# dkogan/mrcal

Hardware: AMD Instinct MI355X
Metric: LM (dog-leg) iterations/sec, 8-cam x 1000-frame OPENCV8 calibration (higher is better)
Workload: dtype f64; 1 GPU; 8 cameras x 1000 frames x 10x10 corners, LENSMODEL_OPENCV8, all variables optimized, warp + regularization; Nstate=6140, Nmeasurements=1600080, Nnz_J=37200080, parallelism=single GPU

## Files before the change

### mrcal_amd/csrc/kernels.hip

```cpp
#include <hip/hip_runtime.h>
#include <utility>
#include <stdlib.h>
#include "problem.hpp"
#include "device_math.hpp"
#include "lens_models.hpp"
#include "lens_dispatch.hpp"
#include "triangulation.hpp"
#include "kernels.hpp"
#include "dogleg_choose.hpp"
#include "kernels_shared.hpp"

namespace mrcal_amd {

__device__ __forceinline__
void joint_pose_record(double* __restrict__ out,
                       const double* rt_cam,
                       const double* rt_frame)
{
    double R[9], dR[27];
    if(rt_cam == NULL)
    {
        R_from_r_with_grad(R, dR, rt_frame);
        for(int i=0;i<9;i++) out[JOINT_R + i] = R[i];
        for(int i=0;i<3;i++) out[JOINT_T + i] = rt_frame[3+i];
// ... 246 lines not shown
        if(c.skip_eval) return;
        board_prologue_body(P, B, dogleg_trial_state(ca, c), ca.ops[c.ia], nblocks_unpack, nblocks_zero, reg_mode);
    }
    else
    {
        if(opref_skip(R)) return;
        const double* b = opref_get(R).b;
        board_prologue_body(P, B, b, opref_get(R), nblocks_unpack, nblocks_zero, reg_mode);
    }
}


__device__ __forceinline__
int board_csr_to_tile_col(const DeviceProblem& P, bool has_ext, int c, int xy)
{
    const int b1 = P.Ncore_state ? 2 : 0;
    const int b2 = b1 + P.Ndist_state;
    const int b3 = b2 + (has_ext ? 6 : 0);
    const int b4 = b3 + (P.do_optimize_frames ? 6 : 0);
    int col = tile_warp0(P.Ndist) + (c - b4);
    col = (c < b4) ? tile_frame0(P.Ndist) + (c - b3) : col;
    col = (c < b3) ? tile_ext0(P.Ndist)   + (c - b2) : col;
    col = (c < b2) ? 4 + (c - b1)                    : col;
    col = (c < b1) ? 2*c + xy                        : col;
    return col;
}

template<int N>
__device__ __forceinline__ double row_ror_f64(double v)
{
    union { double d; int i[2]; } u; u.d = v;
    u.i[0] = __builtin_amdgcn_update_dpp(0, u.i[0], 0x120 + N, 0xf, 0xf, true);
    u.i[1] = __builtin_amdgcn_update_dpp(0, u.i[1], 0x120 + N, 0xf, 0xf, true);
    return u.d;
}

typedef double d2_t __attribute__((ext_vector_type(2)));
typedef __attribute__((address_space(1))) double gdouble;
typedef __attribute__((address_space(1))) d2_t   gdouble2;

typedef double gram_d2 __attribute__((ext_vector_type(2)));
__device__ __forceinline__ gram_d2 lds_read2_b64_16(unsigned lds_byte_address)
{
    gram_d2 v;
    asm volatile("ds_read2_b64 %0, %1 offset1:16" : "=v"(v) : "v"(lds_byte_address) : "memory");
    return v;
}

template<int K, int KS>
__device__ __forceinline__
void copy_out_full(const double* __restrict__ tile, gdouble* __restrict__ out,
                   int A0, int A1, int B0, int B1, unsigned gofs, int rsub)
{
    constexpr int PAIRS = K/2, R = 64/PAIRS;
    constexpr int NIT   = (64 + 2*R - 1)/(2*R);
    const char* __restrict__ t = reinterpret_cast<const char*>(tile);
#pragma unroll
    for(int it0 = 0; it0 < NIT; it0 += 2)
    {
        d2_t v[4];
#pragma unroll
        for(int q=0;q<4;q++)
        {
            const int it = it0 + (q >> 1), u = q & 1;
            const int rb = it*2*R + u*R;
            if(it >= NIT || rb >= 64) continue;
            const int o  = it*2*R*KS*(int)sizeof(double);
            v[q].x = *reinterpret_cast<const double*>(t + (u ? B0 : A0) + o);
            v[q].y = *reinterpret_cast<const double*>(t + (u ? B1 : A1) + o);
        }
#pragma unroll
        for(int q=0;q<4;q++)
        {
            const int it = it0 + (q >> 1), u = q & 1;
            const int rb = it*2*R + u*R;
            if(it >= NIT || rb >= 64) continue;
            gdouble* __restrict__ o = out + rb*K;
            if(rb + R - 1 < 64)      __builtin_nontemporal_store(v[q], reinterpret_cast<gdouble2*>(&o[gofs]));
            else if(rsub < 64 - rb)  __builtin_nontemporal_store(v[q], reinterpret_cast<gdouble2*>(&o[gofs]));
        }
    }
}

template<int NBLK, int MM> struct GramCand
{
    static constexpr int      c    = gram_cand(NBLK, MM);
    static constexpr GramDesc d    = gram_cand_desc(NBLK, c);
    static constexpr bool     roty = gram_rotated_y(NBLK);
    static constexpr int srcA = (d.kind == GRAM_YY) ? 1 : 0;
    static constexpr int srcB = (d.kind == GRAM_XX) ? 0 : (roty ? 1 : 1 + d.q);
    static constexpr int rotB = (d.kind == GRAM_XX || roty) ? d.q : 0;
};
struct GramRd { double v[4]; };
template<int NBLK, int NACC, int... MM>
__device__ __forceinline__ void gram_mfmas(double (&acc)[NACC], const double (&op)[4][4], std::integer_sequence<int, MM...>)
{
    ((acc[MM] = __builtin_amdgcn_mfma_f64_4x4x4f64(op[GramCand<NBLK,MM>::srcA][0],
                                                   op[GramCand<NBLK,MM>::srcB][GramCand<NBLK,MM>::rotB],
                                                   acc[MM], 0, 0, 0)), ...);
}
template<int NBLK, int NM>
__device__ __forceinline__ void gram_step_ops(double (&acc)[NM], const GramRd& rd)
{
    double op[4][4];
#pragma unroll
    for(int g=0; g<4; g++)
    {
        op[g][0] = rd.v[g];
        op[g][1] = row_ror_f64<12>(op[g][0]);
        op[g][2] = row_ror_f64<8 >(op[g][0]);
        op[g][3] = row_ror_f64<4 >(op[g][0]);
    }
    gram_mfmas<NBLK>(acc, op, std::make_integer_sequence<int, NM>{});
}

__device__ __forceinline__ void permlane32_swap_f64(double& a, double& b)
{
    union { double d; unsigned u[2]; } ua, ub;
    ua.d = a; ub.d = b;
#pragma unroll
    for(int i = 0; i < 2; i++)
    {
        const auto r = __builtin_amdgcn_permlane32_swap(ua.u[i], ub.u[i], false, false);
        ua.u[i] = r[0]; ub.u[i] = r[1];
    }
    a = ua.d; b = ub.d;
}

template<int OFF>
__device__ __forceinline__ double lds_read_b64_at(unsigned lds_byte_address)
{
    double v;
    asm volatile("ds_read_b64 %0, %1 offset:%2" : "=v"(v) : "v"(lds_byte_address), "n"(OFF) : "memory");
    return v;
}

template<int NREAD>
__device__ __forceinline__ void lgkm_wait0(GramRd& a, d2_t& b)
{
    if(NREAD == 2)      asm volatile("s_waitcnt lgkmcnt(0)" : "+v"(a.v[0]), "+v"(a.v[1]), "+v"(b) :: "memory");
    else if(NREAD == 3) asm volatile("s_waitcnt lgkmcnt(0)" : "+v"(a.v[0]), "+v"(a.v[1]), "+v"(a.v[2]), "+v"(b) :: "memory");
    else                asm volatile("s_waitcnt lgkmcnt(0)" : "+v"(a.v[0]), "+v"(a.v[1]), "+v"(a.v[2]), "+v"(a.v[3]), "+v"(b) :: "memory");
}
template<int S, bool FULL, bool STORE, int NBLK, int K, int KS, int NM>
__device__ __forceinline__
void fused_step(double (&acc)[NM], GramRd& cur, const unsigned (&gram_a)[4], unsigned tile_a0,
                gdouble* __restrict__ out, int A0, int A1, int B0, int B1, unsigned gofs, int rsub, int nrows)
{
    if(!FULL && 4*S >= nrows) return;
    constexpr int PAIRS = K/2, R = 64/PAIRS, NGRP = (64 + R - 1)/R;
    constexpr int NREAD = gram_nreads(NBLK);
    constexpr bool have_grp = STORE && S < NGRP;
    constexpr int  u  = S & 1;
    constexpr int  go = (S >> 1)*2*R*KS*(int)sizeof(double);
    constexpr int  rb = S*R;
    GramRd nxt = cur;
    if(S < 15)
    {
        constexpr int so = (S < 15 ? S+1 : 0)*(FULL ? 1 : 4)*KS*(int)sizeof(double);
#pragma unroll
        for(int q=0;q<NREAD;q++) nxt.v[q] = lds_read_b64_at<so>(gram_a[q]);
    }
    d2_t v = {0.0, 0.0};
    if(have_grp)
    {
        v.x = lds_read_b64_at<go>(tile_a0 + (unsigned)(u ? B0 : A0));
        v.y = lds_read_b64_at<go>(tile_a0 + (unsigned)(u ? B1 : A1));
    }
    if(S == 0)
    {
        d2_t none = {0.0, 0.0};
        if(!FULL || !have_grp) lgkm_wait0<NREAD>(cur, none);
        else if(NREAD == 2) asm volatile("s_waitcnt lgkmcnt(4)" : "+v"(cur.v[0]), "+v"(cur.v[1]), "+v"(none) :: "memory");
        else if(NREAD == 3) asm volatile("s_waitcnt lgkmcnt(5)" : "+v"(cur.v[0]), "+v"(cur.v[1]), "+v"(cur.v[2]), "+v"(none) :: "memory");
        else                asm volatile("s_waitcnt lgkmcnt(6)" : "+v"(cur.v[0]), "+v"(cur.v[1]), "+v"(cur.v[2]), "+v"(cur.v[3]), "+v"(none) :: "memory");
    }
    __builtin_amdgcn_sched_barrier(0);
    gram_step_ops<NBLK>(acc, cur);
    __builtin_amdgcn_sched_barrier(0);
    lgkm_wait0<NREAD>(nxt, v);
    if(have_grp)
    {
        gdouble* __restrict__ o = out + rb*K;
        if(FULL)
        {
            if(rb + R - 1 < 64)      __builtin_nontemporal_store(v, reinterpret_cast<gdouble2*>(&o[gofs]));
            else if(rsub < 64 - rb)  __builtin_nontemporal_store(v, reinterpret_cast<gdouble2*>(&o[gofs]));
        }
        else if(rb + rsub < nrows)   __builtin_nontemporal_store(v, reinterpret_cast<gdouble2*>(&o[gofs]));
    }
    __builtin_amdgcn_sched_barrier(0);
    cur = nxt;
}
template<bool FULL, bool STORE, int NBLK, int K, int KS, int NM, int... S>
__device__ __forceinline__
void fused_steps(double (&acc)[NM], GramRd& cur, const unsigned (&gram_a)[4], unsigned tile_a0,
                 gdouble* __restrict__ out, int A0, int A1, int B0, int B1, unsigned gofs, int rsub, int nrows,
                 std::integer_sequence<int, S...>)
{
    (fused_step<S,FULL,STORE,NBLK,K,KS>(acc, cur, gram_a, tile_a0, out, A0, A1, B0, B1, gofs, rsub, nrows), ...);
}
template<bool FULL, bool STORE, int NBLK, int K, int KS, int NM>
__device__ __forceinline__
void gram_copy_fused(double (&acc)[NM], const double* __restrict__ tile, const int (&goffs)[4],
                     gdouble* __restrict__ out, int A0, int A1, int B0, int B1, unsigned gofs, int rsub, int nrows)
{
    constexpr int NREAD = gram_nreads(NBLK);
    static_assert(NREAD >= 2 && NREAD <= 4, "board tiles have 5..8 column blocks");
    const unsigned tile_a0 = (unsigned)(size_t)tile;
    const unsigned row_skew = FULL ? (unsigned)((threadIdx.x >> 4)*15*KS*sizeof(double)) : 0u;
    unsigned gram_a[4];
#pragma unroll
    for(int q=0;q<4;q++) gram_a[q] = tile_a0 + row_skew + (unsigned)(goffs[q < NREAD ? q : 0]*sizeof(double));
    GramRd cur;
#pragma unroll
    for(int q=0;q<4;q++) cur.v[q] = 0.0;
#pragma unroll
    for(int q=0;q<NREAD;q++) cur.v[q] = lds_read_b64_at<0>(gram_a[q]);
    fused_steps<FULL,STORE,NBLK,K,KS>(acc, cur, gram_a, tile_a0, out, A0, A1, B0, B1, gofs, rsub, nrows,
                                std::make_integer_sequence<int, 16>{});
}

#ifdef MRCAL_AMD_DEV
#define ABLATE(P, bits) ((P).debug_ablate & (bits))
#else
#define ABLATE(P, bits) 0
#endif
#ifdef BOARD_TS
#define TS(i) do { ts[i] = clock64(); } while(0)
#define TSACC(i, t0) do { const long long _t = clock64(); ts[i] += _t - (t0); (t0) = _t; } while(0)
#else
#define TS(i)
#define TSACC(i, t0)
#endif

template<int K, int NDIST, int KS, bool HAS_EXT>
__device__ __forceinline__
void copy_out_invariants(int lane, int& A0, int& A1, int& B0, int& B1, unsigned& gofs, int& rsub)
{
    constexpr int PPR = K/2, RPI = 64/PPR, NACT = RPI*PPR;
    constexpr int b1 = 2, b2 = 2 + NDIST, b3 = b2 + (HAS_EXT ? 6 : 0), b4 = b3 + 6;
    const int cl = (lane < NACT) ? lane : lane - NACT;
    rsub = cl / PPR;
    const int c0 = 2*(cl - rsub*PPR);
    auto tcol = [&](int c, int xy) -> int
    {
        int col = tile_warp0(NDIST) + (c - b4);
        col = (c < b4) ? tile_frame0(NDIST) + (c - b3) : col;
        col = (c < b3) ? tile_ext0(NDIST)   + (c - b2) : col;
        col = (c < b2) ? 4 + (c - b1)                  : col;
        col = (c < b1) ? 2*c + xy                      : col;
        return col;
    };
    const int y0 = rsub & 1, y1 = (rsub + RPI) & 1;
    A0 = (rsub*KS       + tcol(c0,   y0))*(int)sizeof(double);
    A1 = (rsub*KS       + tcol(c0+1, y0))*(int)sizeof(double);
    B0 = ((rsub+RPI)*KS + tcol(c0,   y1))*(int)sizeof(double);
    B1 = ((rsub+RPI)*KS + tcol(c0+1, y1))*(int)sizeof(double);
    gofs = (unsigned)(rsub*K + c0);
}

template<int PROJ, int NDIST, bool WITH_J, bool WITH_GRAM, bool ALLOPT, bool STORE_J>
__device__ __forceinline__
void board_observation(const DeviceProblem& P,
                       const OpRef& R,
                       const double* __restrict__ joint,
                       double*       __restrict__ gram,
                       const int iobs, double* __restrict__ lds)
{
    constexpr int EXT0   = 4 + NDIST;
    constexpr int FRAME0 = EXT0 + 6;
    constexpr int WARP0  = FRAME0 + 6;
    constexpr int XCOL   = WARP0 + 2;
    constexpr int NCOLS  = XCOL + 1;
    constexpr int NBLK   = (NCOLS + 3)/4;
    constexpr int NCOLS4 = 4*NBLK;
    constexpr int KS     = NCOLS4 | 1;
    constexpr int NM     = gram_nmfma_blk(NBLK);
    static_assert(NBLK <= 8, "the Gram scheme covers 32 tile columns");

    const int lane = threadIdx.x;
#ifdef BOARD_TS
    long long ts[8] = {0,0,0,0,0,0,0,0};
    const long long wall0 = (long long)wall_clock64();
    TS(0);
#endif
    const int NPTS = P.W*P.H;

    const double* __restrict__ pool      = P.board_pool + (size_t)iobs*NPTS*3;
    const double* __restrict__ jp_global = joint + (size_t)iobs*JOINT_STRIDE;
    const int n3 = 3*NPTS, last = n3 - 1;
    const double j0 = jp_global[lane];
    const double j1 = jp_global[(lane < JOINT_REC - 64) ? 64 + lane : JOINT_REC - 1];
    double v_obs[8];
#pragma unroll
    for(int j=0;j<8;j++)
        if(64*j < n3)
        {
            const int idx = 64*j + lane;
            v_obs[j] = pool[idx < last ? idx : last];
        }

    if(opref_skip(R)) return;
    gdouble* __restrict__ x  = (gdouble*)opref_get(R).x;
    gdouble* __restrict__ Jv = (gdouble*)opref_get(R).Jv;

    const BoardObsMeta m = P.board_meta[iobs];
    const int  k       = m.nnz_per_row;
    const bool has_ext = P.do_optimize_extrinsics && m.icam_extrinsics >= 0;

    double* __restrict__ tile    = lds;
    double* __restrict__ obs_lds = lds + 64*KS;
    double* __restrict__ jp      = obs_lds + ((3*NPTS + 63) & ~63);

    double intr[4 + NDIST];
    double warp0, warp1;
    {
        const double* __restrict__ ip = P.unpacked + (size_t)m.icam_intrinsics*P.Nintrinsics;
#pragma unroll
        for(int i=0;i<4+NDIST;i++) intr[i] = ip[i];
        const double* __restrict__ wp = P.unpacked + (size_t)P.Ncameras_intrinsics*P.Nintrinsics;
        warp0 = wp[0]; warp1 = wp[1];
    }

    const double inv_Wm1 = P.inv_Wm1,   inv_Hm1 = P.inv_Hm1;
    const double inv_fx  = 1.0/intr[0], inv_fy  = 1.0/intr[1];

    constexpr int NREAD = gram_nreads(NBLK);
    int goffs[4];
#pragma unroll
    for(int q=0;q<4;q++) goffs[q] = (lane >> 4)*KS + gram_read_col(NBLK, q < NREAD ? q : 0, lane);
    double acc[NM];
#pragma unroll
    for(int mm=0;mm<NM;mm++) acc[mm] = 0.0;

    const int  pairs_per_row = k >> 1;
    const int  rows_per_iter = (k > 0 && !(k & 1)) ? 64 / pairs_per_row : 0;
    const int  co_nactive    = rows_per_iter*pairs_per_row;
    const bool co_active     = lane < co_nactive;
    const int  co_lane       = co_active ? lane : lane - co_nactive;
    const int  co_rsub       = (rows_per_iter > 0) ? co_lane / pairs_per_row : 0;
    const int  co_c0         = 2*(co_lane - co_rsub*pairs_per_row);
    auto co_tile_cols = [&](int* tx0, int* tx1, int* ty0, int* ty1)
    {
        *tx0 = board_csr_to_tile_col(P, has_ext, co_c0,   0);
        *tx1 = board_csr_to_tile_col(P, has_ext, co_c0+1, 0);
        *ty0 = board_csr_to_tile_col(P, has_ext, co_c0,   1);
        *ty1 = board_csr_to_tile_col(P, has_ext, co_c0+1, 1);
    };
    constexpr int KFULL = 2 + NDIST + 14;
    static_assert(!ALLOPT || (WITH_J && WITH_GRAM && !(KFULL & 1)), "ALLOPT: the fused Gram + copy-out path only");
    const bool co_fast  = ALLOPT || (WITH_J && !(KFULL & 1) && (k == KFULL || k == KFULL - 6));
    int co_A0 = 0, co_A1 = 0, co_B0 = 0, co_B1 = 0;
    unsigned co_gofs = 0;
    int co_rsub_c = 0;
    if(ALLOPT)
    {
        if(has_ext) copy_out_invariants<KFULL,   NDIST, KS, true >(lane, co_A0, co_A1, co_B0, co_B1, co_gofs, co_rsub_c);
        else        copy_out_invariants<KFULL-6, NDIST, KS, false>(lane, co_A0, co_A1, co_B0, co_B1, co_gofs, co_rsub_c);
    }
    else if(co_fast)
    {
        int co_tx0, co_tx1, co_ty0, co_ty1;
        co_tile_cols(&co_tx0, &co_tx1, &co_ty0, &co_ty1);
        const bool y0 = (co_rsub & 1) != 0, y1 = ((co_rsub + rows_per_iter) & 1) != 0;
        co_A0 = (co_rsub*KS                 + (y0 ? co_ty0 : co_tx0))*(int)sizeof(double);
        co_A1 = (co_rsub*KS                 + (y0 ? co_ty1 : co_tx1))*(int)sizeof(double);
        co_B0 = ((co_rsub+rows_per_iter)*KS + (y1 ? co_ty0 : co_tx0))*(int)sizeof(double);
        co_B1 = ((co_rsub+rows_per_iter)*KS + (y1 ? co_ty1 : co_tx1))*(int)sizeof(double);
        co_gofs = (unsigned)(co_rsub*k + co_c0);
    }

#pragma unroll
    for(int j=0;j<8;j++)
        if(64*j < n3)
            obs_lds[64*j + lane] = v_obs[j];
    jp[lane] = j0;
    if(lane < JOINT_REC - 64) jp[64 + lane] = j1;
    for(int base = 512; base < n3; base += 64)
    {
        const int idx = base + lane;
        obs_lds[idx] = pool[idx < last ? idx : last];
    }
    __builtin_amdgcn_wave_barrier();
    if(ABLATE(P, 16)) { if(obs_lds[lane] + intr[0] + warp0 + jp[0] == 12345.678) x[0] = 1.0; return; }

#ifdef BOARD_TS
    TS(1);
    long long tcur = ts[1];
#endif
    for(int pt0 = 0; pt0 < NPTS; pt0 += 64)
    {
        const int  pt    = pt0 + lane;
        const bool valid = pt < NPTS;

        double row[2][NCOLS4];
#pragma unroll
        for(int xy=0;xy<2;xy++)
#pragma unroll
            for(int c=0;c<NCOLS4;c++) row[xy][c] = 0.0;

        {
            const int ptc = valid ? pt : NPTS - 1;
            const int iy = ptc / P.W;
            const int ix = ptc - iy*P.W;
            const double bx = (double)ix * P.spacing;
            const double by = (double)iy * P.spacing;
            double bz = 0.0, dz_dw0 = 0.0, dz_dw1 = 0.0;
            if(ALLOPT || P.has_warp_seed)
            {
                const double xr = (double)ix * inv_Wm1;
                const double yr = (double)iy * inv_Hm1;
                dz_dw0 = 4.0*xr*(1.0 - xr);
                dz_dw1 = 4.0*yr*(1.0 - yr);
// ... 44 lines not shown
#pragma unroll
                        for(int i=0;i<NDIST;i++)
                            row[xy][4+i] = dq_dk[xy][i] * w * SCALE_DISTORTION;
                }
                if(ALLOPT || has_ext)
                {
#pragma unroll
                    for(int l=0;l<3;l++)
                    {
                        double dp[3];
#pragma unroll
                        for(int i=0;i<3;i++)
                            dp[i] =
                                bx*jp[JOINT_MC + 0  + 3*i + l] +
                                by*jp[JOINT_MC + 9  + 3*i + l] +
                                bz*jp[JOINT_MC + 18 + 3*i + l] +
                                jp[JOINT_DTJ_DRC + 3*i + l];
#pragma unroll
                        for(int xy=0;xy<2;xy++)
                        {
                            const double g = dq_dp[xy][0]*dp[0] + dq_dp[xy][1]*dp[1] + dq_dp[xy][2]*dp[2];
                            row[xy][EXT0+l]   = g * w * SCALE_ROTATION_CAMERA;
                            row[xy][EXT0+3+l] = dq_dp[xy][l] * w * SCALE_TRANSLATION_CAMERA;
                        }
                    }
                }
                if(ALLOPT || P.do_optimize_frames)
                {
#pragma unroll
                    for(int l=0;l<3;l++)
                    {
                        double dpr[3], dpt[3];
#pragma unroll
                        for(int i=0;i<3;i++)
                        {
                            dpr[i] =
                                bx*jp[JOINT_MF + 0  + 3*i + l] +
                                by*jp[JOINT_MF + 9  + 3*i + l] +
                                bz*jp[JOINT_MF + 18 + 3*i + l];
                            dpt[i] = jp[JOINT_DTJ_DTF + 3*i + l];
                        }
#pragma unroll
                        for(int xy=0;xy<2;xy++)
                        {
                            const double gr = dq_dp[xy][0]*dpr[0] + dq_dp[xy][1]*dpr[1] + dq_dp[xy][2]*dpr[2];
                            const double gt = dq_dp[xy][0]*dpt[0] + dq_dp[xy][1]*dpt[1] + dq_dp[xy][2]*dpt[2];
                            row[xy][FRAME0+l]   = gr * w * SCALE_ROTATION_FRAME;
                            row[xy][FRAME0+3+l] = gt * w * SCALE_TRANSLATION_FRAME;
                        }
                    }
                }
                if(ALLOPT || P.has_warp_state)
                {
#pragma unroll
                    for(int xy=0;xy<2;xy++)
                    {
                        const double d =
                            dq_dp[xy][0]*jp[JOINT_R + 2] +
                            dq_dp[xy][1]*jp[JOINT_R + 5] +
                            dq_dp[xy][2]*jp[JOINT_R + 8];
                        row[xy][WARP0+0] = (w*SCALE_CALOBJECT_WARP)*(d*dz_dw0);
                        row[xy][WARP0+1] = (w*SCALE_CALOBJECT_WARP)*(d*dz_dw1);
                    }
                }
            }
            if(WITH_GRAM)
            {
                row[0][XCOL] = err.x;
                row[1][XCOL] = err.y;
            }
        }

        if(!WITH_J) continue;
        TSACC(2, tcur);

#pragma unroll
        for(int c=0;c<NCOLS4;c++) permlane32_swap_f64(row[0][c], row[1][c]);
        for(int h = 0; h < 2; h++)
        {
            const int nc    = NPTS - pt0 - 32*h;
            if(nc <= 0) break;
            const int nrows = 2*((nc < 32) ? nc : 32);

            __builtin_amdgcn_wave_barrier();
            {
                double* __restrict__ t0 = tile + (size_t)(2*(lane & 31) + (lane >> 5))*KS;
                if(h == 0)
                {
#pragma unroll
                    for(int c=0;c<NCOLS4;c++) t0[c] = row[0][c];
                    asm volatile("" ::: "memory");
                }
                else
                {
#pragma unroll
                    for(int c=0;c<NCOLS4;c++) t0[c] = row[1][c];
                    asm volatile("" ::: "memory");
                }
            }
            __builtin_amdgcn_wave_barrier();
            TSACC(3, tcur);

            gdouble* __restrict__ out = Jv + m.i_nnz0 + (size_t)(2*(pt0 + 32*h))*k;
            if(ALLOPT || (WITH_GRAM && co_fast && !ABLATE(P, 3)))
            {
                const int  rs    = ALLOPT ? co_rsub_c : co_rsub;
                const bool kfull = ALLOPT ? has_ext : (k == KFULL);
                if(nrows == 64)
                {
                    if(kfull) gram_copy_fused<true,STORE_J,NBLK,KFULL,  KS>(acc, tile, goffs, out, co_A0, co_A1, co_B0, co_B1, co_gofs, rs, 64);
                    else      gram_copy_fused<true,STORE_J,NBLK,KFULL-6,KS>(acc, tile, goffs, out, co_A0, co_A1, co_B0, co_B1, co_gofs, rs, 64);
                }
                else
                {
                    if(kfull) gram_copy_fused<false,STORE_J,NBLK,KFULL,  KS>(acc, tile, goffs, out, co_A0, co_A1, co_B0, co_B1, co_gofs, rs, nrows);
                    else      gram_copy_fused<false,STORE_J,NBLK,KFULL-6,KS>(acc, tile, goffs, out, co_A0, co_A1, co_B0, co_B1, co_gofs, rs, nrows);
                }
                TSACC(5, tcur);
                continue;
            }
            if(STORE_J && !ABLATE(P, 1))
            {
                if(co_fast && nrows == 64)
                {
                    if(k == KFULL) copy_out_full<KFULL,   KS>(tile, out, co_A0, co_A1, co_B0, co_B1, co_gofs, co_rsub);
                    else           copy_out_full<KFULL-6, KS>(tile, out, co_A0, co_A1, co_B0, co_B1, co_gofs, co_rsub);
                }
                else if(rows_per_iter > 0)
                {
                    int co_tx0, co_tx1, co_ty0, co_ty1;
                    co_tile_cols(&co_tx0, &co_tx1, &co_ty0, &co_ty1);
                    if(co_active)
                        for(int r = co_rsub; r < nrows; r += rows_per_iter)
                        {
                            const bool isy = (r & 1) != 0;
                            d2_t v;
                            v.x = tile[r*KS + (isy ? co_ty0 : co_tx0)];
                            v.y = tile[r*KS + (isy ? co_ty1 : co_tx1)];
                            __builtin_nontemporal_store(v, reinterpret_cast<gdouble2*>(&out[r*k + co_c0]));
                        }
                }
                else
                {
                    const int nelem = nrows*k;
                    for(int e = 2*lane; e < nelem; e += 128)
                    {
                        const int r0 = e / k,       c0 = e - r0*k;
                        const int r1 = (e+1) / k,   c1 = (e+1) - r1*k;
                        d2_t v;
                        v.x = tile[r0*KS + board_csr_to_tile_col(P, has_ext, c0, r0 & 1)];
                        v.y = tile[r1*KS + board_csr_to_tile_col(P, has_ext, c1, r1 & 1)];
                        __builtin_nontemporal_store(v, reinterpret_cast<gdouble2*>(&out[e]));
                    }
                }
            }

            TSACC(4, tcur);
            if(WITH_GRAM && !ABLATE(P, 2))
            {
                const int nsteps = (nrows + 3) >> 2;
                for(int s = 0; s < nsteps; s++)
                {
                    GramRd rd;
#pragma unroll
                    for(int q=0;q<4;q++) rd.v[q] = (q < NREAD) ? tile[s*4*KS + goffs[q]] : 0.0;
                    gram_step_ops<NBLK>(acc, rd);
                }
            }
#ifdef BOARD_TS
            { const double dep = acc[0]; asm volatile("" :: "v"(dep)); }
#endif
            TSACC(5, tcur);
        }
    }

    if(WITH_J && WITH_GRAM)
    {
        gdouble* __restrict__ g = (gdouble*)gram + (size_t)iobs*(NM*64);
#pragma unroll
        for(int mm=0;mm<NM;mm++)
            g[mm*64 + lane] = acc[mm];
    }
#ifdef BOARD_TS
    TS(6);
    if(P.debug_ts != NULL && lane == 0)
    {
        long long* o = P.debug_ts + (size_t)iobs*10;
        unsigned hwid;
        asm volatile("s_getreg_b32 %0, hwreg(HW_REG_HW_ID)" : "=s"(hwid));
        unsigned xcc;
        asm volatile("s_getreg_b32 %0, hwreg(HW_REG_XCC_ID)" : "=s"(xcc));
        o[0] = ts[0]; o[1] = ts[1]; o[2] = ts[2]; o[3] = ts[3]; o[4] = ts[4]; o[5] = ts[5]; o[6] = ts[6];
        o[7] = (long long)hwid | ((long long)(xcc & 0xf) << 32);
        o[8] = wall0; o[9] = (long long)wall_clock64();
    }
#endif
}

template<int PROJ, int NDIST, bool WITH_J, bool WITH_GRAM, bool ALLOPT = false, bool STORE_J = true>
__global__ __launch_bounds__(64) __attribute__((amdgpu_waves_per_eu(2)))
void board_kernel(DeviceProblem P,
                  OpRef R,
                  const double* __restrict__ joint,
                  double*       __restrict__ gram)
{
    static_assert(STORE_J || (WITH_J && WITH_GRAM), "without the stream the rows exist for the Gram's sake");
    extern __shared__ __attribute__((aligned(16))) double lds[];
    board_observation<PROJ,NDIST,WITH_J,WITH_GRAM,ALLOPT,STORE_J>(P, R, joint, gram, blockIdx.x, lds);
}

__global__ __launch_bounds__(64)
void board_structure_kernel(DeviceProblem P, int32_t* __restrict__ rowptr, int32_t* __restrict__ colidx)
{
    const int iobs = blockIdx.x;
    const int lane = threadIdx.x;
    const BoardObsMeta m = P.board_meta[iobs];
    const int k     = m.nnz_per_row;
    const int nrows = 2*P.W*P.H;
    const bool has_ext = P.do_optimize_extrinsics && m.icam_extrinsics >= 0;

    for(int r = lane; r < nrows; r += 64)
        rowptr[m.i_meas0 + r] = (int32_t)(m.i_nnz0 + (int64_t)r*k);

    const int64_t nelem = (int64_t)nrows*k;
    for(int64_t e = lane; e < nelem; e += 64)
    {
        const int r  = (int)(e / k);
        int       c  = (int)(e - (int64_t)r*k);
        const int xy = r & 1;
        int col;
        if(P.Ncore_state && c < 2)
            col = m.i_state_intrinsics + xy + 2*c;
        else
        {
            if(P.Ncore_state) c -= 2;
            if(c < P.Ndist_row)
                col = m.i_state_intrinsics + P.Ncore_state + c;
            else
            {
                c -= P.Ndist_row;
                if(has_ext && c < 6)
                    col = m.i_state_extrinsics + c;
                else
                {
                    if(has_ext) c -= 6;
                    if(P.do_optimize_frames && c < 6)
                        col = m.i_state_frame + c;
                    else
// ... 459 lines not shown
```

### mrcal_amd/csrc/problem.hpp

```cpp
#pragma once
#include <hip/hip_runtime.h>
#include <stdint.h>
#include "layout.hpp"
#include "lens_models.hpp"

namespace mrcal_amd {

struct BoardObsMeta
{
    int32_t icam_intrinsics;
    int32_t icam_extrinsics;
    int32_t iframe;
    int32_t nnz_per_row;
    int32_t i_state_intrinsics;
    int32_t i_state_extrinsics;
    int32_t i_state_frame;
    int32_t i_meas0;
    int64_t i_nnz0;
    int64_t _pad;
};
static_assert(sizeof(BoardObsMeta) == 48, "BoardObsMeta layout");

struct PointObsMeta
{
    int32_t icam_intrinsics;
    int32_t icam_extrinsics;
    int32_t i_point;
    int32_t nnz_per_row;
    int32_t i_state_intrinsics;
    int32_t i_state_extrinsics;
    int32_t i_state_point;
    int32_t i_meas0;
    int64_t i_nnz0;
    int64_t _pad;
};
static_assert(sizeof(PointObsMeta) == 48, "PointObsMeta layout");

struct TriPairMeta
{
    int32_t i0, i1;
    int32_t icam_extrinsics0;
    int32_t icam_extrinsics1;
    int32_t i_state_extrinsics0;
    int32_t i_state_extrinsics1;
    int32_t i_meas;
    int32_t _pad;
    int64_t i_nnz0;
};
static_assert(sizeof(TriPairMeta) == 40, "TriPairMeta layout");

enum
{
    JOINT_R       = 0,
    JOINT_T       = 9,
    JOINT_MC      = 12,
    JOINT_DTJ_DRC = 39,
    JOINT_MF      = 48,
    JOINT_DTJ_DTF = 75,
    JOINT_REC     = 84,
    JOINT_STRIDE  = 112
};

__host__ __device__ inline int tile_ext0  (int ndist) { return 4 + ndist; }
__host__ __device__ inline int tile_frame0(int ndist) { return 4 + ndist + 6; }
__host__ __device__ inline int tile_warp0 (int ndist) { return 4 + ndist + 12; }
__host__ __device__ inline int tile_xcol  (int ndist) { return 4 + ndist + 14; }
__host__ __device__ inline int tile_ncols (int ndist) { return 4 + ndist + 15; }
__host__ __device__ inline int tile_nblk  (int ndist) { return (tile_ncols(ndist) + 3) >> 2; }
__host__ __device__ inline int tile_stride(int ndist) { return (4*tile_nblk(ndist)) | 1; }

enum { GRAM_XX = 0, GRAM_YY, GRAM_XY };
struct GramDesc { int kind, q; };
__host__ __device__ constexpr int  gram_nx(int nblk) { return nblk < 4 ? nblk : 4; }
__host__ __device__ constexpr int  gram_ny(int nblk) { return nblk - gram_nx(nblk); }
__host__ __device__ constexpr bool gram_rotated_y(int nblk) { return gram_ny(nblk) == 4; }
__host__ __device__ constexpr int  gram_nreads(int nblk) { return 1 + (gram_rotated_y(nblk) ? 1 : gram_ny(nblk)); }
__host__ __device__ constexpr int  gram_ncand(int nblk)
{
    const int ny = gram_ny(nblk);
    if(ny == 0) return 3;
    if(ny == 4) return 3 + 3 + 4;
    return 3 + (ny >= 2 ? 2 : 1) + ny;
}
__host__ __device__ constexpr GramDesc gram_cand_desc(int nblk, int c)
{
    const int ny  = gram_ny(nblk);
    const int nyy = (ny == 4) ? 3 : (ny >= 2 ? 2 : (ny == 1 ? 1 : 0));
    if(c < 3)       return GramDesc{ GRAM_XX, c };
    if(c < 3 + nyy) return GramDesc{ GRAM_YY, c - 3 };
    return GramDesc{ GRAM_XY, c - 3 - nyy };
}
__host__ __device__ constexpr bool gram_slot_pair(int nblk, int c, int s, int* bA, int* bB)
{
    const int nx = gram_nx(nblk), ny = gram_ny(nblk);
    const GramDesc d = gram_cand_desc(nblk, c);
    int a = 0, b = 0;
    bool ok = true;
    if(d.kind == GRAM_XX)
    {
        a = s; b = (s + d.q) & 3;
        ok = a < nx && b < nx && !(d.q == 2 && s >= 2);
    }
    else if(ny == 4)
    {
        b = 4 + ((s + d.q) & 3);
        if(d.kind == GRAM_YY) { a = 4 + s; ok = !(d.q == 2 && s >= 2); }
        else                  { a = s;     ok = a < nx; }
    }
    else if(d.kind == GRAM_XY)
    {
        a = s; b = 4 + (s + d.q) % ny;
        ok = a < nx;
    }
    else
    {
        a = 4 + s % ny; b = 4 + (s + d.q) % ny;
        ok = s < ny && (d.q == 0 || ny == 3 || s == 0);
    }
    *bA = a; *bB = b;
    return ok;
}
__host__ __device__ constexpr bool gram_cand_valid(int nblk, int c)
{
    int a = 0, b = 0;
    return gram_slot_pair(nblk,c,0,&a,&b) || gram_slot_pair(nblk,c,1,&a,&b) ||
           gram_slot_pair(nblk,c,2,&a,&b) || gram_slot_pair(nblk,c,3,&a,&b);
}
__host__ __device__ constexpr int gram_nmfma_blk(int nblk)
{
    int n = 0;
    for(int c = 0; c < gram_ncand(nblk); c++) if(gram_cand_valid(nblk, c)) n++;
    return n;
}
__host__ __device__ constexpr int gram_cand(int nblk, int m)
{
    for(int c = 0; c < gram_ncand(nblk); c++)
        if(gram_cand_valid(nblk, c)) { if(m == 0) return c; m--; }
    return -1;
}
__host__ __device__ inline int gram_stride(int ndist) { return gram_nmfma_blk(tile_nblk(ndist))*64; }
__host__ __device__ inline bool gram_pos_to_entry(int nblk, int pos, int* i, int* j, bool* diag)
{
    const int lane = pos & 63, s = (lane >> 2) & 3;
    const int c = gram_cand(nblk, pos >> 6);
    int bA = 0, bB = 0;
    if(c < 0 || !gram_slot_pair(nblk, c, s, &bA, &bB)) return false;
    *i = 4*bA + (lane >> 4);
    *j = 4*bB + (lane & 3);
    *diag = (bA == bB);
    return true;
}
__host__ __device__ inline int gram_read_col(int nblk, int iread, int lane)
{
    if(iread == 0) return lane & 15;
    const int ny = gram_ny(nblk), s = (lane >> 2) & 3;
    if(ny == 4) return 16 + (lane & 15);
    return 16 + 4*((s + (iread - 1)) % ny) + (lane & 3);
}

struct DeviceProblem
{
    int lens_type;
    int Nintrinsics, Ncore, Ncore_state, Ndist, Ndist_state, Nintr_state;
    int Ndist_row;
    int i_state_intrinsics, i_state_extrinsics, i_state_frames, i_state_points, i_state_warp;
    int Nstate, Nmeas;
    int do_optimize_extrinsics, do_optimize_frames;
    int elim_extrinsics;
    int has_warp_state;
    int has_warp_seed;
    int Ncameras_intrinsics, Ncameras_extrinsics, Nframes, Npoints, Npoints_fixed;
    int Nobs_board, Nobs_point;
    int W, H;
    double spacing;
    double inv_Wm1, inv_Hm1;
    double seed_warp[2];

    LensConfig cfg;

#ifdef MRCAL_AMD_DEV
    int debug_ablate;
    long long* debug_ts;
#endif

    int do_apply_regularization;
    int has_unity_cam01;
    int i_meas_regularization;
    int64_t i_nnz_regularization;
    double imager_width_cam0;

    const double* seed_intrinsics;
    const double* seed_rt_cam_ref;
    const double* seed_rt_ref_frame;
    const double* seed_points;

    const BoardObsMeta* board_meta;
    const double*       board_pool;
    const PointObsMeta* point_meta;
    const double*       point_pool;
    int                 Npairs_tri;
    const TriPairMeta*  tri_meta;
    const double*       tri_px;
    const int*          tri_outlier;
    const int*          imagersizes;

    const double*       unpacked;
};

bool dropin_inputs_ok(mrcal_problem_selections_t problem_selections,
                      const mrcal_observation_point_triangulated_t* observations_point_triangulated,
                      int Nobservations_point_triangulated,
                      int Nobservations_board, const mrcal_calobject_warp_t* calobject_warp,
                      bool warp_seed_first);

}
```

Measured before the change: 8229 iterations/s.

## Replace gram candidate scheme with explicit per-NBLK MFMA operand packing tables

Replaces the generic XX/YY/XY candidate enumeration for the in-register Gram (JtJ) accumulation with hand-built per-block-count packing tables. Each table lists LDS reads, row rotations and which operand pairs feed each f64 4x4x4 MFMA, so some tile widths use fewer MFMAs or fewer wasted slots. LDS addresses are now precomputed from packed 4-bit block indices, and the wait counter is generalized to a variable number of reads. The gain depends on OPENCV8's block count. The risk is correctness of the hand-written tables and extra reads for widths 6 and 7.

```diff
diff --git a/mrcal_amd/csrc/kernels.hip b/mrcal_amd/csrc/kernels.hip
--- a/mrcal_amd/csrc/kernels.hip
+++ b/mrcal_amd/csrc/kernels.hip
@@ -352,36 +352,80 @@
     }
 }
 
-template<int NBLK, int MM> struct GramCand
-{
-    static constexpr int      c    = gram_cand(NBLK, MM);
-    static constexpr GramDesc d    = gram_cand_desc(NBLK, c);
-    static constexpr bool     roty = gram_rotated_y(NBLK);
-    static constexpr int srcA = (d.kind == GRAM_YY) ? 1 : 0;
-    static constexpr int srcB = (d.kind == GRAM_XX) ? 0 : (roty ? 1 : 1 + d.q);
-    static constexpr int rotB = (d.kind == GRAM_XX || roty) ? d.q : 0;
+template<int NBLK> struct GramPack
+{
+    static constexpr int NOP   = gram_packing(NBLK).nop;
+    static constexpr int NREAD = gram_nreads(NBLK);
+    static constexpr int NM    = gram_nmfma_blk(NBLK);
 };
-struct GramRd { double v[4]; };
-template<int NBLK, int NACC, int... MM>
-__device__ __forceinline__ void gram_mfmas(double (&acc)[NACC], const double (&op)[4][4], std::integer_sequence<int, MM...>)
-{
-    ((acc[MM] = __builtin_amdgcn_mfma_f64_4x4x4f64(op[GramCand<NBLK,MM>::srcA][0],
-                                                   op[GramCand<NBLK,MM>::srcB][GramCand<NBLK,MM>::rotB],
+template<int NBLK, int O> struct GramOp
+{
+    static constexpr int src = gram_packing(NBLK).op[O].src, rot = gram_packing(NBLK).op[O].rot;
+    static constexpr int b0  = gram_packing(NBLK).op[O].blk[0], b1 = gram_packing(NBLK).op[O].blk[1];
+    static constexpr int b2  = gram_packing(NBLK).op[O].blk[2], b3 = gram_packing(NBLK).op[O].blk[3];
+};
+template<int NBLK, int MM> struct GramMfmaOps
+{
+    static constexpr int a = gram_packing(NBLK).mfma[MM].a, b = gram_packing(NBLK).mfma[MM].b;
+};
+template<int N> struct GramRd { double v[N]; };
+template<int NBLK, int O, int NOP, int NREAD>
+__device__ __forceinline__ void gram_operand(double (&op)[NOP], const GramRd<NREAD>& rd)
+{
+    using o = GramOp<NBLK,O>;
+    if constexpr(o::src < 0)
+    {
+        static_assert(O < NREAD, "the reads come first");
+        op[O] = rd.v[O];
+    }
+    else
+    {
+        static_assert(o::src < O && o::rot >= 1 && o::rot <= 3, "a rotation follows its source");
+        op[O] = row_ror_f64<16 - 4*o::rot>(op[o::src]);
+    }
+}
+template<int NBLK, int NOP, int NREAD, int... O>
+__device__ __forceinline__ void gram_operands(double (&op)[NOP], const GramRd<NREAD>& rd, std::integer_sequence<int, O...>)
+{
+    (gram_operand<NBLK,O>(op, rd), ...);
+}
+template<int NBLK, int NACC, int NOP, int... MM>
+__device__ __forceinline__ void gram_mfmas(double (&acc)[NACC], const double (&op)[NOP], std::integer_sequence<int, MM...>)
+{
+    ((acc[MM] = __builtin_amdgcn_mfma_f64_4x4x4f64(op[GramMfmaOps<NBLK,MM>::a],
+                                                   op[GramMfmaOps<NBLK,MM>::b],
                                                    acc[MM], 0, 0, 0)), ...);
 }
-template<int NBLK, int NM>
-__device__ __forceinline__ void gram_step_ops(double (&acc)[NM], const GramRd& rd)
-{
-    double op[4][4];
-#pragma unroll
-    for(int g=0; g<4; g++)
-    {
-        op[g][0] = rd.v[g];
-        op[g][1] = row_ror_f64<12>(op[g][0]);
-        op[g][2] = row_ror_f64<8 >(op[g][0]);
-        op[g][3] = row_ror_f64<4 >(op[g][0]);
-    }
+template<int NBLK, int NM, int NREAD>
+__device__ __forceinline__ void gram_step_ops(double (&acc)[NM], const GramRd<NREAD>& rd)
+{
+    constexpr int NOP = GramPack<NBLK>::NOP;
+    static_assert(NM == GramPack<NBLK>::NM && NREAD == GramPack<NBLK>::NREAD, "the packing's sizes");
+    double op[NOP];
+    gram_operands<NBLK>(op, rd, std::make_integer_sequence<int, NOP>{});
     gram_mfmas<NBLK>(acc, op, std::make_integer_sequence<int, NM>{});
+}
+template<int NBLK, int... Q>
+__device__ __forceinline__ unsigned gram_slot_blocks(int s, std::integer_sequence<int, Q...>)
+{
+    constexpr unsigned p0 = (((unsigned)GramOp<NBLK,Q>::b0 << (4*Q)) | ...), p1 = (((unsigned)GramOp<NBLK,Q>::b1 << (4*Q)) | ...);
+    constexpr unsigned p2 = (((unsigned)GramOp<NBLK,Q>::b2 << (4*Q)) | ...), p3 = (((unsigned)GramOp<NBLK,Q>::b3 << (4*Q)) | ...);
+    return s == 0 ? p0 : s == 1 ? p1 : s == 2 ? p2 : p3;
+}
+template<int NREAD>
+__device__ __forceinline__ void gram_full_addresses(unsigned (&a)[NREAD], unsigned base, unsigned blocks)
+{
+    static_assert(NREAD <= 8, "4 bits a read");
+#pragma unroll
+    for(int q=0;q<NREAD;q++) a[q] = base + (((blocks >> (4*q)) & 0xfu) << 5);
+}
+template<int KS, int NREAD>
+__device__ __forceinline__ void gram_partial_addresses(unsigned (&a)[NREAD], const unsigned (&full)[NREAD])
+{
+    unsigned skew = (unsigned)((threadIdx.x >> 4)*15*KS*sizeof(double));
+    asm volatile("" : "+v"(skew));
+#pragma unroll
+    for(int q=0;q<NREAD;q++) a[q] = full[q] - skew;
 }
 
 __device__ __forceinline__ void permlane32_swap_f64(double& a, double& b)
@@ -405,26 +449,27 @@
     return v;
 }
 
-template<int NREAD>
-__device__ __forceinline__ void lgkm_wait0(GramRd& a, d2_t& b)
-{
-    if(NREAD == 2)      asm volatile("s_waitcnt lgkmcnt(0)" : "+v"(a.v[0]), "+v"(a.v[1]), "+v"(b) :: "memory");
-    else if(NREAD == 3) asm volatile("s_waitcnt lgkmcnt(0)" : "+v"(a.v[0]), "+v"(a.v[1]), "+v"(a.v[2]), "+v"(b) :: "memory");
-    else                asm volatile("s_waitcnt lgkmcnt(0)" : "+v"(a.v[0]), "+v"(a.v[1]), "+v"(a.v[2]), "+v"(a.v[3]), "+v"(b) :: "memory");
-}
-template<int S, bool FULL, bool STORE, int NBLK, int K, int KS, int NM>
+template<int N, int NREAD>
+__device__ __forceinline__ void lgkm_wait(GramRd<NREAD>& a, d2_t& b)
+{
+    static_assert(N >= 0 && N <= 15, "lgkmcnt is a 4-bit counter");
+    asm volatile("s_waitcnt lgkmcnt(%0)" :: "n"(N) : "memory");
+#pragma unroll
+    for(int q=0;q<NREAD;q++) asm volatile("" : "+v"(a.v[q]));
+    asm volatile("" : "+v"(b));
+}
+template<int S, bool FULL, bool STORE, int NBLK, int K, int KS, int NM, int NREAD>
 __device__ __forceinline__
-void fused_step(double (&acc)[NM], GramRd& cur, const unsigned (&gram_a)[4], unsigned tile_a0,
+void fused_step(double (&acc)[NM], GramRd<NREAD>& cur, const unsigned (&gram_a)[NREAD], unsigned tile_a0,
                 gdouble* __restrict__ out, int A0, int A1, int B0, int B1, unsigned gofs, int rsub, int nrows)
 {
     if(!FULL && 4*S >= nrows) return;
     constexpr int PAIRS = K/2, R = 64/PAIRS, NGRP = (64 + R - 1)/R;
-    constexpr int NREAD = gram_nreads(NBLK);
     constexpr bool have_grp = STORE && S < NGRP;
     constexpr int  u  = S & 1;
     constexpr int  go = (S >> 1)*2*R*KS*(int)sizeof(double);
     constexpr int  rb = S*R;
-    GramRd nxt = cur;
+    GramRd<NREAD> nxt = cur;
     if(S < 15)
     {
         constexpr int so = (S < 15 ? S+1 : 0)*(FULL ? 1 : 4)*KS*(int)sizeof(double);
@@ -440,15 +485,13 @@
     if(S == 0)
     {
         d2_t none = {0.0, 0.0};
-        if(!FULL || !have_grp) lgkm_wait0<NREAD>(cur, none);
-        else if(NREAD == 2) asm volatile("s_waitcnt lgkmcnt(4)" : "+v"(cur.v[0]), "+v"(cur.v[1]), "+v"(none) :: "memory");
-        else if(NREAD == 3) asm volatile("s_waitcnt lgkmcnt(5)" : "+v"(cur.v[0]), "+v"(cur.v[1]), "+v"(cur.v[2]), "+v"(none) :: "memory");
-        else                asm volatile("s_waitcnt lgkmcnt(6)" : "+v"(cur.v[0]), "+v"(cur.v[1]), "+v"(cur.v[2]), "+v"(cur.v[3]), "+v"(none) :: "memory");
+        if(!FULL || !have_grp) lgkm_wait<0>(cur, none);
+        else                   lgkm_wait<NREAD + 2>(cur, none);
     }
     __builtin_amdgcn_sched_barrier(0);
     gram_step_ops<NBLK>(acc, cur);
     __builtin_amdgcn_sched_barrier(0);
-    lgkm_wait0<NREAD>(nxt, v);
+    lgkm_wait<0>(nxt, v);
     if(have_grp)
     {
         gdouble* __restrict__ o = out + rb*K;
@@ -462,29 +505,29 @@
     __builtin_amdgcn_sched_barrier(0);
     cur = nxt;
 }
-template<bool FULL, bool STORE, int NBLK, int K, int KS, int NM, int... S>
+template<bool FULL, bool STORE, int NBLK, int K, int KS, int NM, int NREAD, int... S>
 __device__ __forceinline__
-void fused_steps(double (&acc)[NM], GramRd& cur, const unsigned (&gram_a)[4], unsigned tile_a0,
+void fused_steps(double (&acc)[NM], GramRd<NREAD>& cur, const unsigned (&gram_a)[NREAD], unsigned tile_a0,
                  gdouble* __restrict__ out, int A0, int A1, int B0, int B1, unsigned gofs, int rsub, int nrows,
                  std::integer_sequence<int, S...>)
 {
     (fused_step<S,FULL,STORE,NBLK,K,KS>(acc, cur, gram_a, tile_a0, out, A0, A1, B0, B1, gofs, rsub, nrows), ...);
 }
-template<bool FULL, bool STORE, int NBLK, int K, int KS, int NM>
+template<bool FULL, bool STORE, int NBLK, int K, int KS, int NM, int NREAD>
 __device__ __forceinline__
-void gram_copy_fused(double (&acc)[NM], const double* __restrict__ tile, const int (&goffs)[4],
+void gram_copy_fused(double (&acc)[NM], const double* __restrict__ tile, const unsigned (&gram_full)[NREAD],
                      gdouble* __restrict__ out, int A0, int A1, int B0, int B1, unsigned gofs, int rsub, int nrows)
 {
-    constexpr int NREAD = gram_nreads(NBLK);
-    static_assert(NREAD >= 2 && NREAD <= 4, "board tiles have 5..8 column blocks");
+    static_assert(NREAD >= 2 && NREAD <= 8, "a k-step's requests and the copy-out's two fit the wait counter");
     const unsigned tile_a0 = (unsigned)(size_t)tile;
-    const unsigned row_skew = FULL ? (unsigned)((threadIdx.x >> 4)*15*KS*sizeof(double)) : 0u;
-    unsigned gram_a[4];
-#pragma unroll
-    for(int q=0;q<4;q++) gram_a[q] = tile_a0 + row_skew + (unsigned)(goffs[q < NREAD ? q : 0]*sizeof(double));
-    GramRd cur;
-#pragma unroll
-    for(int q=0;q<4;q++) cur.v[q] = 0.0;
+    unsigned gram_a[NREAD];
+    if(FULL)
+    {
+#pragma unroll
+        for(int q=0;q<NREAD;q++) gram_a[q] = gram_full[q];
+    }
+    else gram_partial_addresses<KS>(gram_a, gram_full);
+    GramRd<NREAD> cur;
 #pragma unroll
     for(int q=0;q<NREAD;q++) cur.v[q] = lds_read_b64_at<0>(gram_a[q]);
     fused_steps<FULL,STORE,NBLK,K,KS>(acc, cur, gram_a, tile_a0, out, A0, A1, B0, B1, gofs, rsub, nrows,
@@ -597,9 +640,8 @@
     const double inv_fx  = 1.0/intr[0], inv_fy  = 1.0/intr[1];
 
     constexpr int NREAD = gram_nreads(NBLK);
-    int goffs[4];
-#pragma unroll
-    for(int q=0;q<4;q++) goffs[q] = (lane >> 4)*KS + gram_read_col(NBLK, q < NREAD ? q : 0, lane);
+    const unsigned gram_base   = (unsigned)(size_t)tile + (unsigned)(((lane >> 4)*16*KS + (lane & 3))*sizeof(double));
+    unsigned       gram_blocks = gram_slot_blocks<NBLK>((lane >> 2) & 3, std::make_integer_sequence<int, NREAD>{});
     double acc[NM];
 #pragma unroll
     for(int mm=0;mm<NM;mm++) acc[mm] = 0.0;
@@ -810,6 +852,10 @@
             if(nc <= 0) break;
             const int nrows = 2*((nc < 32) ? nc : 32);
 
+            if(!ALLOPT) asm volatile("" : "+v"(gram_blocks));
+            unsigned gram_full[NREAD];
+            gram_full_addresses(gram_full, gram_base, gram_blocks);
+
             __builtin_amdgcn_wave_barrier();
             {
                 double* __restrict__ t0 = tile + (size_t)(2*(lane & 31) + (lane >> 5))*KS;
@@ -836,13 +882,13 @@
                 const bool kfull = ALLOPT ? has_ext : (k == KFULL);
                 if(nrows == 64)
                 {
-                    if(kfull) gram_copy_fused<true,STORE_J,NBLK,KFULL,  KS>(acc, tile, goffs, out, co_A0, co_A1, co_B0, co_B1, co_gofs, rs, 64);
-                    else      gram_copy_fused<true,STORE_J,NBLK,KFULL-6,KS>(acc, tile, goffs, out, co_A0, co_A1, co_B0, co_B1, co_gofs, rs, 64);
+                    if(kfull) gram_copy_fused<true,STORE_J,NBLK,KFULL,  KS>(acc, tile, gram_full, out, co_A0, co_A1, co_B0, co_B1, co_gofs, rs, 64);
+                    else      gram_copy_fused<true,STORE_J,NBLK,KFULL-6,KS>(acc, tile, gram_full, out, co_A0, co_A1, co_B0, co_B1, co_gofs, rs, 64);
                 }
                 else
                 {
-                    if(kfull) gram_copy_fused<false,STORE_J,NBLK,KFULL,  KS>(acc, tile, goffs, out, co_A0, co_A1, co_B0, co_B1, co_gofs, rs, nrows);
-                    else      gram_copy_fused<false,STORE_J,NBLK,KFULL-6,KS>(acc, tile, goffs, out, co_A0, co_A1, co_B0, co_B1, co_gofs, rs, nrows);
+                    if(kfull) gram_copy_fused<false,STORE_J,NBLK,KFULL,  KS>(acc, tile, gram_full, out, co_A0, co_A1, co_B0, co_B1, co_gofs, rs, nrows);
+                    else      gram_copy_fused<false,STORE_J,NBLK,KFULL-6,KS>(acc, tile, gram_full, out, co_A0, co_A1, co_B0, co_B1, co_gofs, rs, nrows);
                 }
                 TSACC(5, tcur);
                 continue;
@@ -887,11 +933,14 @@
             if(WITH_GRAM && !ABLATE(P, 2))
             {
                 const int nsteps = (nrows + 3) >> 2;
+                unsigned gram_a[NREAD];
+                gram_partial_addresses<KS>(gram_a, gram_full);
+                typedef __attribute__((address_space(3))) const double lds_cdouble;
                 for(int s = 0; s < nsteps; s++)
                 {
-                    GramRd rd;
-#pragma unroll
-                    for(int q=0;q<4;q++) rd.v[q] = (q < NREAD) ? tile[s*4*KS + goffs[q]] : 0.0;
+                    GramRd<NREAD> rd;
+#pragma unroll
+                    for(int q=0;q<NREAD;q++) rd.v[q] = reinterpret_cast<lds_cdouble*>(gram_a[q])[s*4*KS];
                     gram_step_ops<NBLK>(acc, rd);
                 }
             }
diff --git a/mrcal_amd/csrc/problem.hpp b/mrcal_amd/csrc/problem.hpp
--- a/mrcal_amd/csrc/problem.hpp
+++ b/mrcal_amd/csrc/problem.hpp
@@ -69,82 +69,119 @@
 __host__ __device__ inline int tile_nblk  (int ndist) { return (tile_ncols(ndist) + 3) >> 2; }
 __host__ __device__ inline int tile_stride(int ndist) { return (4*tile_nblk(ndist)) | 1; }
 
-enum { GRAM_XX = 0, GRAM_YY, GRAM_XY };
-struct GramDesc { int kind, q; };
-__host__ __device__ constexpr int  gram_nx(int nblk) { return nblk < 4 ? nblk : 4; }
-__host__ __device__ constexpr int  gram_ny(int nblk) { return nblk - gram_nx(nblk); }
-__host__ __device__ constexpr bool gram_rotated_y(int nblk) { return gram_ny(nblk) == 4; }
-__host__ __device__ constexpr int  gram_nreads(int nblk) { return 1 + (gram_rotated_y(nblk) ? 1 : gram_ny(nblk)); }
-__host__ __device__ constexpr int  gram_ncand(int nblk)
-{
-    const int ny = gram_ny(nblk);
-    if(ny == 0) return 3;
-    if(ny == 4) return 3 + 3 + 4;
-    return 3 + (ny >= 2 ? 2 : 1) + ny;
-}
-__host__ __device__ constexpr GramDesc gram_cand_desc(int nblk, int c)
-{
-    const int ny  = gram_ny(nblk);
-    const int nyy = (ny == 4) ? 3 : (ny >= 2 ? 2 : (ny == 1 ? 1 : 0));
-    if(c < 3)       return GramDesc{ GRAM_XX, c };
-    if(c < 3 + nyy) return GramDesc{ GRAM_YY, c - 3 };
-    return GramDesc{ GRAM_XY, c - 3 - nyy };
-}
-__host__ __device__ constexpr bool gram_slot_pair(int nblk, int c, int s, int* bA, int* bB)
-{
-    const int nx = gram_nx(nblk), ny = gram_ny(nblk);
-    const GramDesc d = gram_cand_desc(nblk, c);
-    int a = 0, b = 0;
-    bool ok = true;
-    if(d.kind == GRAM_XX)
-    {
-        a = s; b = (s + d.q) & 3;
-        ok = a < nx && b < nx && !(d.q == 2 && s >= 2);
-    }
-    else if(ny == 4)
-    {
-        b = 4 + ((s + d.q) & 3);
-        if(d.kind == GRAM_YY) { a = 4 + s; ok = !(d.q == 2 && s >= 2); }
-        else                  { a = s;     ok = a < nx; }
-    }
-    else if(d.kind == GRAM_XY)
-    {
-        a = s; b = 4 + (s + d.q) % ny;
-        ok = a < nx;
-    }
-    else
-    {
-        a = 4 + s % ny; b = 4 + (s + d.q) % ny;
-        ok = s < ny && (d.q == 0 || ny == 3 || s == 0);
-    }
-    *bA = a; *bB = b;
-    return ok;
-}
-__host__ __device__ constexpr bool gram_cand_valid(int nblk, int c)
-{
-    int a = 0, b = 0;
-    return gram_slot_pair(nblk,c,0,&a,&b) || gram_slot_pair(nblk,c,1,&a,&b) ||
-           gram_slot_pair(nblk,c,2,&a,&b) || gram_slot_pair(nblk,c,3,&a,&b);
-}
-__host__ __device__ constexpr int gram_nmfma_blk(int nblk)
-{
+enum { GRAM_MAXOP = 10, GRAM_MAXMFMA = 10 };
+struct GramOperand
+{
+    int blk[4];
+    int src, rot;
+};
+struct GramMfma { int a, b, valid; };
+struct GramPacking
+{
+    int nop, nmfma;
+    GramOperand op[GRAM_MAXOP];
+    GramMfma    mfma[GRAM_MAXMFMA];
+};
+__host__ __device__ constexpr void gram_add_read(GramPacking& p, int b0, int b1, int b2, int b3)
+{
+    p.op[p.nop++] = GramOperand{ {b0, b1, b2, b3}, -1, 0 };
+}
+__host__ __device__ constexpr void gram_add_rot(GramPacking& p, int src, int rot)
+{
+    const GramOperand& o = p.op[src];
+    p.op[p.nop++] = GramOperand{ {o.blk[rot & 3], o.blk[(1+rot) & 3], o.blk[(2+rot) & 3], o.blk[(3+rot) & 3]}, src, rot };
+}
+__host__ __device__ constexpr void gram_add_mfma(GramPacking& p, int a, int b, int valid = 0xf)
+{
+    p.mfma[p.nmfma++] = GramMfma{ a, b, valid };
+}
+__host__ __device__ constexpr GramPacking gram_packing(int nblk)
+{
+    GramPacking p{};
+    if(nblk == 5)
+    {
+        gram_add_read(p, 0,1,2,3);
+        gram_add_read(p, 4,4,4,4);
+        gram_add_rot (p, 0, 1);
+        gram_add_rot (p, 0, 2);
+        gram_add_mfma(p, 0, 0);
+        gram_add_mfma(p, 0, 2);
+        gram_add_mfma(p, 0, 3, 0x3);
+        gram_add_mfma(p, 1, 1, 0x1);
+        gram_add_mfma(p, 0, 1);
+    }
+    else if(nblk == 6)
+    {
+        gram_add_read(p, 0,1,2,3);
+        gram_add_read(p, 1,2,3,0);
+        gram_add_read(p, 4,5,4,5);
+        gram_add_read(p, 5,4,5,4);
+        gram_add_read(p, 0,1,4,5);
+        gram_add_read(p, 2,3,4,5);
+        gram_add_mfma(p, 0, 0);
+        gram_add_mfma(p, 0, 1);
+        gram_add_mfma(p, 0, 2);
+        gram_add_mfma(p, 0, 3);
+        gram_add_mfma(p, 4, 5);
+        gram_add_mfma(p, 2, 3, 0x1);
+    }
+    else if(nblk == 7)
+    {
+        gram_add_read(p, 0,1,2,3);
+        gram_add_read(p, 1,2,3,0);
+        gram_add_read(p, 4,5,6,4);
+        gram_add_read(p, 5,6,4,5);
+        gram_add_read(p, 6,4,5,6);
+        gram_add_read(p, 4,6,4,5);
+        gram_add_read(p, 0,1,5,6);
+        gram_add_read(p, 2,3,5,6);
+        gram_add_mfma(p, 0, 0);
+        gram_add_mfma(p, 0, 1);
+        gram_add_mfma(p, 0, 2);
+        gram_add_mfma(p, 0, 3);
+        gram_add_mfma(p, 0, 4);
+        gram_add_mfma(p, 2, 5);
+        gram_add_mfma(p, 6, 7);
+    }
+    else if(nblk == 8)
+    {
+        gram_add_read(p, 0,1,2,3);
+        gram_add_read(p, 4,5,6,7);
+        gram_add_rot (p, 0, 1);
+        gram_add_rot (p, 0, 2);
+        gram_add_rot (p, 1, 1);
+        gram_add_rot (p, 1, 2);
+        gram_add_rot (p, 1, 3);
+        gram_add_mfma(p, 0, 0);
+        gram_add_mfma(p, 0, 2);
+        gram_add_mfma(p, 0, 3, 0x3);
+        gram_add_mfma(p, 1, 1);
+        gram_add_mfma(p, 1, 4);
+        gram_add_mfma(p, 1, 5, 0x3);
+        gram_add_mfma(p, 0, 1);
+        gram_add_mfma(p, 0, 4);
+        gram_add_mfma(p, 0, 5);
+        gram_add_mfma(p, 0, 6);
+    }
+    return p;
+}
+__host__ __device__ constexpr int gram_nreads(int nblk)
+{
+    const GramPacking p = gram_packing(nblk);
     int n = 0;
-    for(int c = 0; c < gram_ncand(nblk); c++) if(gram_cand_valid(nblk, c)) n++;
+    for(int o = 0; o < p.nop; o++) if(p.op[o].src < 0) n++;
     return n;
 }
-__host__ __device__ constexpr int gram_cand(int nblk, int m)
-{
-    for(int c = 0; c < gram_ncand(nblk); c++)
-        if(gram_cand_valid(nblk, c)) { if(m == 0) return c; m--; }
-    return -1;
-}
+__host__ __device__ constexpr int gram_nmfma_blk(int nblk) { return nblk == 8 ? 10 : (nblk >= 5 && nblk <= 7) ? nblk : 0; }
+static_assert(gram_packing(5).nmfma == gram_nmfma_blk(5) && gram_packing(6).nmfma == gram_nmfma_blk(6) &&
+              gram_packing(7).nmfma == gram_nmfma_blk(7) && gram_packing(8).nmfma == gram_nmfma_blk(8), "gram_nmfma_blk()");
 __host__ __device__ inline int gram_stride(int ndist) { return gram_nmfma_blk(tile_nblk(ndist))*64; }
 __host__ __device__ inline bool gram_pos_to_entry(int nblk, int pos, int* i, int* j, bool* diag)
 {
-    const int lane = pos & 63, s = (lane >> 2) & 3;
-    const int c = gram_cand(nblk, pos >> 6);
-    int bA = 0, bB = 0;
-    if(c < 0 || !gram_slot_pair(nblk, c, s, &bA, &bB)) return false;
+    const GramPacking p = gram_packing(nblk);
+    const int lane = pos & 63, s = (lane >> 2) & 3, m = pos >> 6;
+    if(m >= p.nmfma || !((p.mfma[m].valid >> s) & 1)) return false;
+    const int bA = p.op[p.mfma[m].a].blk[s], bB = p.op[p.mfma[m].b].blk[s];
     *i = 4*bA + (lane >> 4);
     *j = 4*bB + (lane & 3);
     *diag = (bA == bB);
@@ -152,10 +189,7 @@
 }
 __host__ __device__ inline int gram_read_col(int nblk, int iread, int lane)
 {
-    if(iread == 0) return lane & 15;
-    const int ny = gram_ny(nblk), s = (lane >> 2) & 3;
-    if(ny == 4) return 16 + (lane & 15);
-    return 16 + 4*((s + (iread - 1)) % ny) + (lane & 3);
+    return 4*gram_packing(nblk).op[iread].blk[(lane >> 2) & 3] + (lane & 3);
 }
 
 struct DeviceProblem
```

Measured after the change: 8462 iterations/s (median of 6 runs). +2.8%, better.
